# a-slide/Quade

Hardware: AMD Instinct MI355X
Metric: read-pairs/sec demultiplexed (2x150 bp, dual 8 bp index) (higher is better)
Workload: dtype u8

## Files before the change

### quade_amd/csrc/quade_deflate.hip

```cpp
#include <hip/hip_runtime.h>
#include <stdint.h>
#include <stdio.h>

#include "crc_lds.h"
#include "quade_deflate.h"

namespace {
constexpr int BLOCK = 256, TILE = BLOCK * 16;
constexpr uint32_t HEADER_BITS = 80 + 3 + 14 + 19 * 3 + 259 * 4;

__device__ uint32_t rev_bits(uint32_t v, int n) { return __brev(v) >> (32 - n); }

__device__ void code_lengths(const uint32_t* freq, int n, uint8_t* len, uint16_t* order , uint32_t* w , int16_t* parent ) {
    int m = 0;
    for (int s = 0; s < n; ++s) {
        len[s] = 0;
        if (freq[s]) order[m++] = (uint16_t)s;
    }
    for (int s = 0; m < 2 && s < n; ++s) {
        bool used = false;
        for (int i = 0; i < m; ++i) used |= order[i] == s;
        if (!used) order[m++] = (uint16_t)s;
    }
    auto f = [&](int s) -> uint32_t { return freq[s] ? freq[s] : 1u; };
    for (int i = 1; i < m; ++i) {
        const uint16_t s = order[i];
        int j = i - 1;
        while (j >= 0 && (f(order[j]) > f(s) || (f(order[j]) == f(s) && order[j] > s))) {
            order[j + 1] = order[j];
            --j;
        }
        order[j + 1] = s;
    }
    for (int i = 0; i < m; ++i) w[i] = f(order[i]);
    for (int i = 0; i < 2 * m - 1; ++i) parent[i] = -1;
    int leaf = 0, inner = m, next = m;
    while (next < 2 * m - 1) {
        int pick[2];
        for (int k = 0; k < 2; ++k) pick[k] = (leaf < m && (inner >= next || w[leaf] <= w[inner])) ? leaf++ : inner++;
        w[next] = w[pick[0]] + w[pick[1]];
        parent[pick[0]] = parent[pick[1]] = (int16_t)next;
        ++next;
    }
    int bl[16] = {0};
    w[2 * m - 2] = 0;
    for (int k = 2 * m - 3; k >= 0; --k) w[k] = w[parent[k]] + 1;
    for (int i = 0; i < m; ++i) ++bl[w[i] < 15 ? w[i] : 15];
    uint32_t kraft = 0;
    for (int d = 1; d <= 15; ++d) kraft += (uint32_t)bl[d] << (15 - d);
    for (uint32_t excess = kraft - (1u << 15); excess > 0; --excess) {
        int bits = 14;
        while (bl[bits] == 0) --bits;
        --bl[bits];
        bl[bits + 1] += 2;
        --bl[15];
    }
    int at = 0;
    for (int bits = 15; bits >= 1; --bits)
        for (int c = 0; c < bl[bits]; ++c) len[order[at++]] = (uint8_t)bits;
}

__global__ __launch_bounds__(BLOCK) void huff_pieces(const uint8_t* text, const qd_deflate_piece* pieces, uint8_t* out,
                                                     int64_t out_stride, uint32_t* out_bytes) {
    __shared__ uint32_t hist[4][4][256];
    __shared__ uint32_t freq[257];
    __shared__ uint32_t lut[257];
    __shared__ uint8_t len[257];
    __shared__ uint16_t order[257];
    __shared__ uint32_t wtmp[513];
    __shared__ int16_t parent[513];
    __shared__ uint32_t scan[BLOCK];
    __shared__ uint32_t words[TILE * 15 / 32 + 16];
    __shared__ uint32_t carry_word, carry_bits;
    const int tid = threadIdx.x, wave = tid >> 6, rep = tid & 3;
    const int64_t a = (int64_t)pieces[blockIdx.x].text_off, L = (int64_t)pieces[blockIdx.x].text_len;
    const uint8_t* src = text + a;
    uint32_t* dst = reinterpret_cast<uint32_t*>(out + (int64_t)blockIdx.x * out_stride);
    for (int i = tid; i < 4 * 4 * 256; i += BLOCK) (&hist[0][0][0])[i] = 0;
    __syncthreads();
    for (int64_t t = 0; t < L; t += TILE) {
        const int64_t p = t + (int64_t)tid * 16;
        if (p + 16 <= L) {
            const uint4 v = *reinterpret_cast<const uint4*>(src + p);
            const uint32_t q[4] = {v.x, v.y, v.z, v.w};
#pragma unroll
            for (int j = 0; j < 16; ++j) atomicAdd(&hist[wave][rep][(q[j >> 2] >> (8 * (j & 3))) & 0xff], 1u);
        } else {
            for (int64_t i = p; i < L; ++i) atomicAdd(&hist[wave][rep][src[i]], 1u);
        }
    }
    __syncthreads();
    for (int s = tid; s < 256; s += BLOCK) {
        uint32_t c = 0;
        for (int i = 0; i < 16; ++i) c += (&hist[0][0][0])[i * 256 + s];
        freq[s] = c;
    }
    if (tid == 0) freq[256] = 1;
    __syncthreads();
    if (tid == 0) {
        code_lengths(freq, 257, len, order, wtmp, parent);
        int blc[16] = {0}, nxt[16] = {0};
        for (int s = 0; s < 257; ++s) ++blc[len[s]];
        blc[0] = 0;
        for (int b = 1, c = 0; b <= 15; ++b) {
            c = (c + blc[b - 1]) << 1;
            nxt[b] = c;
        }
        for (int s = 0; s < 257; ++s) lut[s] = len[s] ? ((uint32_t)len[s] | (rev_bits((uint32_t)nxt[len[s]]++, len[s]) << 8)) : 0;
        uint64_t acc = 0;
        int cnt = 0, wi = 0;
        auto put = [&](uint32_t v, int n) {
            acc |= (uint64_t)v << cnt;
            cnt += n;
            if (cnt >= 32) {
                dst[wi++] = (uint32_t)acc;
                acc >>= 32;
                cnt -= 32;
            }
        };
        const uint8_t head[10] = {0x1f, 0x8b, 8, 0, 0, 0, 0, 0, 0, 0xff};
        for (int i = 0; i < 10; ++i) put(head[i], 8);
        put(1, 1);
        put(2, 2);
        put(0, 5);
        put(1, 5);
        put(15, 4);
        const uint8_t ord[19] = {16, 17, 18, 0, 8, 7, 9, 6, 10, 5, 11, 4, 12, 3, 13, 2, 14, 1, 15};
        for (int k = 0; k < 19; ++k) put(ord[k] < 16 ? 4 : 0, 3);
        for (int s = 0; s < 257; ++s) put(rev_bits(len[s], 4), 4);
        put(rev_bits(1, 4), 4);
        put(rev_bits(1, 4), 4);
        carry_word = (uint32_t)acc;
        carry_bits = (uint32_t)cnt;
        scan[0] = (uint32_t)wi;
        uint64_t bits = HEADER_BITS;
        for (int s = 0; s < 257; ++s) bits += (uint64_t)freq[s] * len[s];
        scan[1] = ((bits + 7) / 8 + 8 + 8 <= (uint64_t)out_stride) ? 1u : 0u;
    }
    __syncthreads();
    uint32_t out_word = scan[0];
    const bool fits = scan[1] != 0;
    __syncthreads();
    if (!fits) {
        if (tid == 0) out_bytes[blockIdx.x] = 0;
        return;
    }
    for (int64_t t = 0; t < L; t += TILE) {
        const int64_t p = t + (int64_t)tid * 16;
        uint32_t q[4] = {0, 0, 0, 0};
        int nbytes = 0;
        if (p + 16 <= L) {
            const uint4 v = *reinterpret_cast<const uint4*>(src + p);
            q[0] = v.x; q[1] = v.y; q[2] = v.z; q[3] = v.w;
            nbytes = 16;
        } else if (p < L) {
            nbytes = (int)(L - p);
            for (int i = 0; i < nbytes; ++i) q[i >> 2] |= (uint32_t)src[p + i] << (8 * (i & 3));
        }
        uint64_t b[4] = {0, 0, 0, 0};
        uint32_t nb = 0;
#pragma unroll
        for (int j = 0; j < 16; ++j) {
            if (j < nbytes) {
                const uint32_t e = lut[(q[j >> 2] >> (8 * (j & 3))) & 0xff];
                const uint64_t c = e >> 8;
                const uint32_t l = e & 0xff, wi = nb >> 6, sh = nb & 63;
                b[wi] |= c << sh;
                if (sh + l > 64 && wi < 3) b[wi + 1] |= c >> (64 - sh);
                nb += l;
            }
        }
        uint32_t x = nb;
#pragma unroll
        for (int d = 1; d < 64; d <<= 1) {
            const uint32_t y = __shfl_up(x, d, 64);
            if ((tid & 63) >= d) x += y;
        }
        if ((tid & 63) == 63) scan[wave] = x;
        __syncthreads();
        uint32_t base = 0, total = 0;
#pragma unroll
        for (int i = 0; i < BLOCK / 64; ++i) {
            const uint32_t v = scan[i];
            if (i < wave) base += v;
            total += v;
        }
        const uint32_t mine = base + x - nb;
        const uint32_t cb = carry_bits, cw = carry_word;
        const uint32_t nwords = (cb + total + 31) >> 5;
        for (uint32_t i = tid; i <= nwords; i += BLOCK) words[i] = i == 0 ? cw : 0;
        __syncthreads();
        if (nb) {
            const uint32_t pos = cb + mine, w0 = pos >> 5, sh = pos & 31;
            uint32_t prev = 0;
#pragma unroll
            for (int i = 0; i < 8; ++i) {
                const uint32_t d = (uint32_t)(b[i >> 1] >> (32 * (i & 1)));
                const uint32_t o = sh ? (d << sh) | (prev >> (32 - sh)) : d;
                if (o && 32u * i < nb + sh) atomicOr(&words[w0 + i], o);
                prev = d;
            }
            const uint32_t o = sh ? prev >> (32 - sh) : 0;
            if (o) atomicOr(&words[w0 + 8], o);
        }
        __syncthreads();
        const uint32_t full = (cb + total) >> 5;
        for (uint32_t i = tid; i < full; i += BLOCK) dst[out_word + i] = words[i];
        __syncthreads();
        if (tid == 0) {
            carry_word = words[full];
            carry_bits = (cb + total) & 31;
        }
        out_word += full;
        __syncthreads();
    }
    if (tid == 0) {
        uint64_t acc = carry_word;
        int cnt = (int)carry_bits;
        const uint32_t e = lut[256];
        acc |= (uint64_t)(e >> 8) << cnt;
        cnt += (int)(e & 0xff);
        uint8_t* bytes = reinterpret_cast<uint8_t*>(dst) + (size_t)out_word * 4;
        int nby = 0;
        while (cnt > 0) {
            bytes[nby++] = (uint8_t)acc;
            acc >>= 8;
            cnt -= 8;
        }
        const uint32_t c = pieces[blockIdx.x].crc32, isz = (uint32_t)L;
        for (int i = 0; i < 4; ++i) bytes[nby++] = (uint8_t)(c >> (8 * i));
        for (int i = 0; i < 4; ++i) bytes[nby++] = (uint8_t)(isz >> (8 * i));
        out_bytes[blockIdx.x] = out_word * 4 + (uint32_t)nby;
    }
}

}

hipError_t qd_launch_huffman(const uint8_t* text, const qd_deflate_piece* pieces, uint32_t n_pieces, uint8_t* out, int64_t out_stride,
                             uint32_t* out_bytes, hipStream_t st) {
    if (n_pieces == 0) return hipSuccess;
    hipLaunchKernelGGL(huff_pieces, dim3(n_pieces), dim3(BLOCK), 0, st, text, pieces, out, out_stride, out_bytes);
    return hipGetLastError();
}

namespace {
#ifndef QD_LZ_WAVES
#define QD_LZ_WAVES 8
#endif
constexpr int LZ_SUB = QD_LZ_SUB, LZ_WAVES = QD_LZ_WAVES, LZ_BLOCK = 64 * LZ_WAVES, LZ_REG = LZ_SUB / LZ_WAVES;
constexpr int LZ_HASH_BITS = 11, LZ_NICE = 32, LZ_DNA_MIN = 12, LZ_MATCH_BITS = 13, LZ_MAXLEN = 256;
constexpr int LZ_CRC_SW = LZ_WAVES >= 16 ? 17 : (LZ_WAVES >= 8 ? 33 : 65);
constexpr int LZ_TEXT_WORDS = (LZ_SUB + 320) / 4;
constexpr int LZ_NL = 286, LZ_ND = 30;
static_assert(LZ_SUB <= 65536 && LZ_SUB % 256 == 0, "table entries are 16-bit positions inside the sub-block");

__device__ __forceinline__ uint32_t rd32(const uint32_t* tw, uint32_t p) {
    const uint32_t i = p >> 2;
    return __builtin_amdgcn_alignbyte(tw[i + 1], tw[i], p & 3u);
}
__device__ __forceinline__ void rd256(const uint32_t* tw, uint32_t p, uint32_t (&a)[8]) {
    const uint32_t i = p >> 2, sh = p & 3u;
    uint32_t w[9];
#pragma unroll
    for (int k = 0; k < 9; ++k) w[k] = tw[i + k];
#pragma unroll
    for (int k = 0; k < 8; ++k) a[k] = __builtin_amdgcn_alignbyte(w[k + 1], w[k], sh);
}
__device__ __forceinline__ uint32_t same32(const uint32_t* tw, const uint32_t (&a)[8], uint32_t c) {
    uint32_t b[8];
    rd256(tw, c, b);
    uint32_t n = 32;
#pragma unroll
    for (int k = 7; k >= 0; --k) {
        const uint32_t x = a[k] ^ b[k];
        if (x) n = 4u * (uint32_t)k + ((uint32_t)__builtin_ctz(x) >> 3);
    }
    return n;
}
__device__ __forceinline__ bool bases4(uint32_t v) {
    return __builtin_amdgcn_perm(0x4E000000u, 0x47544341u, (v >> 1) & 0x07070707u) == v;
}
__device__ __forceinline__ void len_symbol(uint32_t l, uint32_t& sym, uint32_t& eb, uint32_t& ev) {
    if (l < 8) {
        sym = 257 + l;
        eb = ev = 0;
    } else if (l == 255) {
        sym = 285;
        eb = ev = 0;
    } else {
        const uint32_t n = 31u - (uint32_t)__clz(l);
        eb = n - 2;
        sym = 257 + 4 * (n - 1) + ((l >> eb) & 3u);
        ev = l & ((1u << eb) - 1);
    }
}
__device__ __forceinline__ void dist_symbol(uint32_t d, uint32_t& sym, uint32_t& eb, uint32_t& ev) {
    if (d < 4) {
        sym = d;
        eb = ev = 0;
    } else {
        const uint32_t n = 31u - (uint32_t)__clz(d);
        eb = n - 1;
        sym = 2 * n + ((d >> eb) & 1u);
        ev = d & ((1u << eb) - 1);
    }
}
__device__ __forceinline__ uint32_t len_extra_bits(uint32_t sym) {
    return (sym < 265 || sym == 285) ? 0u : (sym - 261) >> 2;
}
__device__ __forceinline__ uint32_t dist_extra_bits(uint32_t sym) { return sym < 4 ? 0u : (sym >> 1) - 1; }

__device__ void block_code_lengths(const uint32_t* freq, int n, uint8_t* len, uint32_t* fx, uint16_t* order, uint32_t* w, int16_t* parent,
                                   uint32_t* m_out) {
    __shared__ uint32_t bl[16];
    const int tid = threadIdx.x, nthr = blockDim.x;
    for (int s = tid; s < n; s += nthr) {
        fx[s] = freq[s];
        len[s] = 0;
    }
    if (tid < 16) bl[tid] = 0;
    if (tid == 0) *m_out = 0;
    __syncthreads();
    for (int s = tid; s < n; s += nthr)
        if (fx[s]) atomicAdd(m_out, 1u);
    __syncthreads();
    if (tid == 0 && *m_out < 2) {
        int used = (int)*m_out;
        for (int s = 0; used < 2 && s < n; ++s)
            if (!fx[s]) {
                fx[s] = 1;
                ++used;
            }
        *m_out = (uint32_t)used;
    }
    __syncthreads();
    const int m = (int)*m_out;
    for (int s = tid; s < n; s += nthr) {
        const uint32_t f = fx[s];
        if (!f) continue;
        int rank = 0;
        for (int t = 0; t < n; ++t) {
            const uint32_t g = fx[t];
            rank += (g != 0 && (g < f || (g == f && t < s))) ? 1 : 0;
        }
        order[rank] = (uint16_t)s;
        w[rank] = f;
    }
    for (int i = tid; i < 2 * m - 1; i += nthr) parent[i] = -1;
    __syncthreads();
    if (tid == 0) {
        int leaf = 0, inner = m, next = m;
        while (next < 2 * m - 1) {
            int pick[2];
            for (int k = 0; k < 2; ++k) pick[k] = (leaf < m && (inner >= next || w[leaf] <= w[inner])) ? leaf++ : inner++;
            w[next] = w[pick[0]] + w[pick[1]];
            parent[pick[0]] = parent[pick[1]] = (int16_t)next;
            ++next;
        }
    }
    __syncthreads();
    for (int i = tid; i < m; i += nthr) {
        uint32_t d = 0;
        for (int k = i; parent[k] >= 0; k = parent[k]) ++d;
        atomicAdd(&bl[d < 15 ? d : 15], 1u);
    }
    __syncthreads();
    if (tid == 0) {
        uint32_t kraft = 0;
        for (int d = 1; d <= 15; ++d) kraft += bl[d] << (15 - d);
        for (uint32_t excess = kraft - (1u << 15); excess > 0; --excess) {
            int bits = 14;
            while (bl[bits] == 0) --bits;
            --bl[bits];
            bl[bits + 1] += 2;
            --bl[15];
        }
    }
    __syncthreads();
    for (int i = tid; i < m; i += nthr) {
        int bits = 15;
        for (uint32_t upto = bl[15]; (uint32_t)i >= upto && bits > 1;) upto += bl[--bits];
        len[order[i]] = (uint8_t)bits;
    }
    __syncthreads();
}

__device__ void block_canonical_lut(const uint8_t* len, int n, uint32_t* lut) {
    __shared__ uint32_t cnt[16], nxt[16];
    const int tid = threadIdx.x, nthr = blockDim.x;
    if (tid < 16) cnt[tid] = 0;
    __syncthreads();
    for (int s = tid; s < n; s += nthr)
        if (len[s]) atomicAdd(&cnt[len[s]], 1u);
    __syncthreads();
    if (tid == 0) {
        uint32_t c = 0;
        for (int b = 1; b <= 15; ++b) {
            c = (c + (b > 1 ? cnt[b - 1] : 0u)) << 1;
            nxt[b] = c;
        }
    }
    __syncthreads();
    for (int s = tid; s < n; s += nthr) {
        const uint32_t l = len[s];
        uint32_t rank = 0;
        for (int t = 0; t < s; ++t) rank += len[t] == l ? 1u : 0u;
        lut[s] = l ? (l | (rev_bits(nxt[l] + rank, (int)l) << 8)) : 0u;
    }
    __syncthreads();
}

__device__ __forceinline__ void lds_barrier() { asm volatile("s_waitcnt lgkmcnt(0)\n\ts_barrier" ::: "memory"); }

#if defined(QD_LZ_TIMING)
__device__ unsigned long long g_lz_ticks[8];
#define LZ_STAMP(k)                                                          \
    do {                                                                     \
        __syncthreads();                                                     \
        const uint64_t now_ = (uint64_t)wall_clock64();                      \
        if (threadIdx.x == 0) atomicAdd(&g_lz_ticks[k], (unsigned long long)(now_ - since_)); \
        since_ = now_;                                                       \
    } while (0)
#else
#define LZ_STAMP(k) \
    do {            \
    } while (0)
#endif

__global__ __launch_bounds__(LZ_BLOCK) void lz_subblocks(const uint8_t* text, const qd_lz_sub* subs, uint32_t* tokens, uint8_t* sub_out,
                                                         int64_t sub_stride, uint32_t* sub_bytes, uint32_t* sub_crc) {
    extern __shared__ __attribute__((aligned(16))) uint8_t lz_lds[];
    uint32_t* tw = reinterpret_cast<uint32_t*>(lz_lds);
    uint32_t* table = reinterpret_cast<uint32_t*>(lz_lds + (size_t)LZ_TEXT_WORDS * 4);
    __shared__ uint32_t lfreq[288], dfreq[32], llut[288], dlut[32];
    __shared__ uint8_t llen[288], dlen[32], bcost[256];
    __shared__ uint32_t wave_ntok[LZ_WAVES], scan[LZ_WAVES], ctl[4];
    __shared__ uint32_t carry_word, carry_bits;
    const uint32_t tid = threadIdx.x, lane = tid & 63u, wave = tid >> 6;
    const uint32_t L = subs[blockIdx.x].text_len;
    const uint8_t* src = text + subs[blockIdx.x].text_off;
    uint32_t* dst = reinterpret_cast<uint32_t*>(sub_out + (int64_t)blockIdx.x * sub_stride);
    uint32_t* tok0 = tokens + (size_t)blockIdx.x * LZ_SUB;
#if defined(QD_LZ_TIMING)
    uint64_t since_ = (uint64_t)wall_clock64();
#endif

    static_assert((1u << LZ_HASH_BITS) == 8 * 256, "the byte histogram's replicas borrow the hash table's space");
    for (uint32_t i = tid; i < (1u << LZ_HASH_BITS); i += LZ_BLOCK) table[i] = 0;
    for (uint32_t i = tid; i < 288; i += LZ_BLOCK) lfreq[i] = 0;
    if (tid < 32) dfreq[tid] = 0;
    __syncthreads();
    for (uint32_t i = tid; i < (uint32_t)LZ_TEXT_WORDS / 4; i += LZ_BLOCK) {
        uint4 v = make_uint4(0, 0, 0, 0);
        const uint32_t b = i * 16;
        if (b + 16 <= L) {
            v = *reinterpret_cast<const uint4*>(src + b);
        } else if (b < L) {
            uint32_t q[4] = {0, 0, 0, 0};
            for (uint32_t k = b; k < L; ++k) q[(k - b) >> 2] |= (uint32_t)src[k] << (8 * ((k - b) & 3));
            v = make_uint4(q[0], q[1], q[2], q[3]);
        }
        reinterpret_cast<uint4*>(tw)[i] = v;
        if (b < L) {
            const uint32_t q[4] = {v.x, v.y, v.z, v.w}, nby = min(16u, L - b);
            uint32_t* rep = table + (tid & 7u);
#pragma unroll
            for (uint32_t k = 0; k < 16; ++k)
                if (k < nby) atomicAdd(&rep[((q[k >> 2] >> (8 * (k & 3))) & 0xFFu) << 3], 1u);
        }
    }
    __syncthreads();
    if (tid < 256) {
        uint32_t h = 0;
#pragma unroll
        for (int r = 0; r < 8; ++r) h += table[(tid << 3) + r];
        const int c = h ? (int)(__log2f((float)L / (float)h) + 0.5f) : 12;
        bcost[tid] = (uint8_t)(c < 1 ? 1 : (c > 12 ? 12 : c));
    }
    __syncthreads();
    LZ_STAMP(0);
    if (sub_crc) {
        static_assert((4u << LZ_HASH_BITS) >= 4096 + 64 && (size_t)LZ_BLOCK * LZ_CRC_SW * 4 >= (size_t)LZ_SUB, "the CRC stage's tables and slices");
        qdcrc::stage_tables<LZ_BLOCK>(table);
        __syncthreads();
        const uint32_t crc = qdcrc::crc32_lds<LZ_BLOCK, LZ_CRC_SW>(tw, L, table, table + 1024);
        if (tid == 0) sub_crc[blockIdx.x] = crc;
    }
    for (uint32_t i = tid; i < (1u << LZ_HASH_BITS); i += LZ_BLOCK) table[i] = 0;
    __syncthreads();
    LZ_STAMP(1);

    for (uint32_t r0 = 0; r0 < L; r0 += LZ_BLOCK) {
        const uint32_t p = r0 + tid;
        uint32_t ins_h = 0xFFFFFFFFu, ins_v = 0;
        if (p < L) {
            uint32_t a[8];
            rd256(tw, p, a);
            uint32_t best = 0, dist = 0;
            if (p + 4 <= L) {
                const uint32_t h = (a[0] * 2654435761u) >> (32 - LZ_HASH_BITS);
                const uint32_t bucket = table[h];
                if (p >= 1 && rd32(tw, p - 1) == a[0]) {
                    best = same32(tw, a, p - 1);
                    dist = 1;
                }
#pragma unroll
                for (int k = 0; k < 2; ++k) {
                    const uint32_t c = (bucket >> (16 * k)) & 0xFFFFu;
                    uint32_t n = 0;
                    if (c < p && rd32(tw, c) == a[0]) n = same32(tw, a, c);
                    if (c < p && p - c <= 32768u && n > best) {
                        best = n;
                        dist = p - c;
                    }
                }
                best = min(best, L - p);
                const uint32_t need = (bases4(a[0]) && bases4(a[1])) ? (uint32_t)LZ_DNA_MIN : 4u;
                if (best < need) {
                    best = 0;
                } else {
                    uint32_t c8 = 0;
#pragma unroll
                    for (int k = 0; k < 8; ++k) c8 += bcost[(a[k >> 2] >> (8 * (k & 3))) & 0xFFu];
                    const uint32_t mbits = (uint32_t)LZ_MATCH_BITS + (dist > 1 ? 31u - (uint32_t)__clz(dist) : 0u);
                    if (best * c8 < mbits * 8) best = 0;
                }
#if defined(QD_LZ_RACY)
                table[h] = (bucket << 16) | p;
#else
                ins_h = h;
                ins_v = (bucket << 16) | p;
#endif
            }
            tok0[p] = best | (dist << 8);
        }
        lds_barrier();
#if !defined(QD_LZ_RACY)
        if (ins_h != 0xFFFFFFFFu) atomicMax(&table[ins_h], ins_v);
        lds_barrier();
#endif
    }
    __syncthreads();

    LZ_STAMP(2);
    {
        const uint32_t rbeg = wave * LZ_REG, rend = min(rbeg + (uint32_t)LZ_REG, L);
        uint32_t* tok = tok0 + rbeg;
        uint32_t ntok = 0;
        int carry = 0;
        constexpr uint32_t AHEAD = (1u << LZ_HASH_BITS) / LZ_WAVES / 64;
        static_assert(AHEAD >= 1 && AHEAD * 64 * LZ_WAVES == (1u << LZ_HASH_BITS), "the waves' shares of the table's space");
        uint32_t* cbuf = table + wave * (AHEAD * 64);
        uint32_t in_buf = AHEAD;
        for (uint32_t base = rbeg; base < rend; base += 64) {
            const uint32_t p = base + lane;
            const int limit = (int)min(64u, rend - base);
            uint32_t eff = 0, dist = 0;
            if (in_buf == AHEAD) {
#pragma unroll
                for (uint32_t j = 0; j < AHEAD; ++j) cbuf[64 * j + lane] = p + 64 * j < rend ? tok0[p + 64 * j] : 0u;
                in_buf = 0;
            }
            const uint32_t cd = cbuf[64 * in_buf + lane];
            ++in_buf;
            if ((int)lane < limit) {
                eff = min(cd & 0xFFu, rend - p);
                dist = cd >> 8;
                if (eff < 4) eff = 0;
            }
            const uint32_t lit = (tw[p >> 2] >> (8 * (p & 3u))) & 0xFFu;
            const uint32_t eff_next = (uint32_t)__shfl_down((int)eff, 1, 64);
            const bool deferred = eff != 0 && (int)lane + 1 < limit && eff_next > eff && eff < (uint32_t)LZ_NICE;
            const uint64_t mm = __ballot(eff != 0 && !deferred);
            const uint64_t xm = __ballot(eff >= (uint32_t)LZ_NICE && !deferred);
            uint32_t tlen = eff;
            const uint32_t tdist = dist;
            uint64_t starts = 0;
            int s = carry;
            while (s < limit) {
                if ((mm >> s) & 1ull) {
                    uint32_t len = (uint32_t)__builtin_amdgcn_readlane((int)eff, s);
                    if ((xm >> s) & 1ull) {
                        const uint32_t D = (uint32_t)__builtin_amdgcn_readlane((int)dist, s);
                        const uint32_t ps = base + (uint32_t)s;
                        const uint32_t x = rd32(tw, ps + 4 * lane) ^ rd32(tw, ps - D + 4 * lane);
                        const uint64_t nz = __ballot(x != 0);
                        len = LZ_MAXLEN;
                        if (nz) {
                            const int fl = __builtin_ctzll(nz);
                            const uint32_t xf = (uint32_t)__builtin_amdgcn_readlane((int)x, fl);
                            len = 4u * (uint32_t)fl + ((uint32_t)__builtin_ctz(xf) >> 3);
                        }
                        len = min(len, rend - ps);
                        if ((int)lane == s) tlen = len;
                    }
                    starts |= 1ull << s;
                    s += (int)len;
                } else {
                    const uint64_t rest = (mm >> s) << s;
                    int nxt = rest ? __builtin_ctzll(rest) : 64;
                    if (nxt > limit) nxt = limit;
                    const uint64_t upto = nxt >= 64 ? ~0ull : ((1ull << nxt) - 1);
                    starts |= upto & ~((1ull << s) - 1);
                    s = nxt;
                }
            }
            if (!((mm >> lane) & 1ull)) tlen = 0;
            carry = s - 64;
            if ((starts >> lane) & 1ull) {
                uint32_t t;
                if (tlen) {
                    t = (tlen - 3) | ((tdist - 1) << 8);
                    uint32_t sym, eb, ev;
                    len_symbol(tlen - 3, sym, eb, ev);
                    atomicAdd(&lfreq[sym], 1u);
                    dist_symbol(tdist - 1, sym, eb, ev);
                    atomicAdd(&dfreq[sym], 1u);
                } else {
                    t = 0x80000000u | lit;
                    atomicAdd(&lfreq[lit], 1u);
                }
                tok[ntok + (uint32_t)__popcll(starts & ((1ull << lane) - 1))] = t;
            }
            ntok += (uint32_t)__popcll(starts);
        }
        if (lane == 0) wave_ntok[wave] = ntok;
    }
    if (tid == 0) lfreq[256] = 1;
    __syncthreads();
    LZ_STAMP(3);

    {
        uint32_t* fx = tw;
        uint16_t* order = reinterpret_cast<uint16_t*>(tw + 288);
        uint32_t* w = tw + 288 + 144;
        int16_t* parent = reinterpret_cast<int16_t*>(tw + 288 + 144 + 576);
        block_code_lengths(lfreq, LZ_NL, llen, fx, order, w, parent, &ctl[2]);
        block_code_lengths(dfreq, LZ_ND, dlen, fx, order, w, parent, &ctl[2]);
    }
    LZ_STAMP(4);
    uint32_t* words = tw + 2048;
    block_canonical_lut(llen, LZ_NL, llut);
    block_canonical_lut(dlen, LZ_ND, dlut);
    if (tid == 0) ctl[3] = 0;
    __syncthreads();
    {
        uint32_t bits = 0;
        for (uint32_t s = tid; s < (uint32_t)LZ_NL; s += LZ_BLOCK) bits += lfreq[s] * (llen[s] + (s > 256 ? len_extra_bits(s) : 0u));
        for (uint32_t s = tid; s < (uint32_t)LZ_ND; s += LZ_BLOCK) bits += dfreq[s] * (dlen[s] + dist_extra_bits(s));
        if (bits) atomicAdd(&ctl[3], bits);
    }
    __syncthreads();
    LZ_STAMP(7);
    if (tid == 0) {
        int nl = LZ_NL, nd = LZ_ND;
        while (nl > 257 && llen[nl - 1] == 0) --nl;
        while (nd > 1 && dlen[nd - 1] == 0) --nd;
        uint64_t acc = 0;
        int cnt = 0, wi = 0;
        auto put = [&](uint32_t v, int n) {
            acc |= (uint64_t)v << cnt;
            cnt += n;
            if (cnt >= 32) {
                dst[wi++] = (uint32_t)acc;
                acc >>= 32;
                cnt -= 32;
            }
        };
        put(0, 1);
        put(2, 2);
        put((uint32_t)(nl - 257), 5);
        put((uint32_t)(nd - 1), 5);
        put(15, 4);
        const uint8_t ord[19] = {16, 17, 18, 0, 8, 7, 9, 6, 10, 5, 11, 4, 12, 3, 13, 2, 14, 1, 15};
        for (int k = 0; k < 19; ++k) put(ord[k] == 0 ? 2u : ((ord[k] == 17 || ord[k] == 18) ? 3u : 5u), 3);
        auto len_at = [&](int i) -> uint32_t { return i < nl ? llen[i] : dlen[i - nl]; };
        auto put_len = [&](uint32_t v) { put(rev_bits(15u + v, 5), 5); };
        const int nseq = nl + nd;
        for (int i = 0; i < nseq;) {
            const uint32_t v = len_at(i);
            int run = 1;
            while (i + run < nseq && len_at(i + run) == v) ++run;
            i += run;
            if (v == 0) {
                while (run >= 11) {
                    const int r = run < 138 ? run : 138;
                    put(6, 3);
                    put((uint32_t)(r - 11), 7);
                    run -= r;
                }
                if (run >= 3) {
                    put(2, 3);
                    put((uint32_t)(run - 3), 3);
                    run = 0;
                }
                for (; run > 0; --run) put(0, 2);
            } else {
                put_len(v);
                --run;
                while (run >= 3) {
                    const int r = run < 6 ? run : 6;
                    put_len(16);
                    put((uint32_t)(r - 3), 2);
                    run -= r;
                }
                for (; run > 0; --run) put_len(v);
            }
        }
        carry_word = (uint32_t)acc;
        carry_bits = (uint32_t)cnt;
        const uint64_t bits = 3 + 14 + 19 * 3 + 5 * (uint64_t)(nl + nd) + ctl[3];
        ctl[0] = (uint32_t)wi;
        ctl[1] = ((bits + 7) / 8 + 3 + 4 + 8 <= (uint64_t)sub_stride) ? 1u : 0u;
    }
    __syncthreads();
    LZ_STAMP(5);
    uint32_t out_word = ctl[0];
    if (ctl[1] == 0) {
        if (tid == 0) sub_bytes[blockIdx.x] = 0;
        return;
    }
    constexpr int LZ_TPL = 4;
    uint32_t pre[LZ_WAVES + 1];
    pre[0] = 0;
#pragma unroll
    for (int i = 0; i < LZ_WAVES; ++i) pre[i + 1] = pre[i] + wave_ntok[i];
    const uint32_t T = pre[LZ_WAVES];
    for (uint32_t g0 = 0; g0 < T; g0 += LZ_BLOCK * LZ_TPL) {
        uint32_t t[LZ_TPL];
#pragma unroll
        for (int j = 0; j < LZ_TPL; ++j) {
            const uint32_t g = g0 + tid * LZ_TPL + j;
            t[j] = 0;
            if (g < T) {
                uint32_t wv = 0;
#pragma unroll
                for (int i = 1; i < LZ_WAVES; ++i) wv += g >= pre[i] ? 1u : 0u;
                t[j] = tok0[(size_t)wv * LZ_REG + (g - pre[wv])];
            }
        }
        uint64_t b[LZ_TPL];
        uint32_t nb[LZ_TPL], mine = 0;
#pragma unroll
        for (int j = 0; j < LZ_TPL; ++j) {
            b[j] = 0;
            nb[j] = 0;
            if (g0 + tid * LZ_TPL + j < T) {
                if (t[j] & 0x80000000u) {
                    const uint32_t e = llut[t[j] & 0xFFu];
                    b[j] = e >> 8;
                    nb[j] = e & 0xFFu;
                } else {
                    uint32_t sym, eb, ev;
                    len_symbol(t[j] & 0xFFu, sym, eb, ev);
                    uint32_t e = llut[sym];
                    b[j] = (uint64_t)(e >> 8) | ((uint64_t)ev << (e & 0xFFu));
                    nb[j] = (e & 0xFFu) + eb;
                    dist_symbol((t[j] >> 8) & 0x7FFFu, sym, eb, ev);
                    e = dlut[sym];
                    b[j] |= ((uint64_t)(e >> 8) | ((uint64_t)ev << (e & 0xFFu))) << nb[j];
                    nb[j] += (e & 0xFFu) + eb;
                }
            }
            mine += nb[j];
        }
        uint32_t x = mine;
#pragma unroll
        for (int d = 1; d < 64; d <<= 1) {
            const uint32_t y = __shfl_up(x, d, 64);
            if (lane >= (uint32_t)d) x += y;
        }
        if (lane == 63) scan[wave] = x;
        lds_barrier();
        uint32_t before = 0, total = 0;
#pragma unroll
        for (int i = 0; i < LZ_WAVES; ++i) {
            const uint32_t v = scan[i];
            if ((uint32_t)i < wave) before += v;
            total += v;
        }
        const uint32_t cb = carry_bits, cw = carry_word;
        const uint32_t nwords = (cb + total + 31) >> 5;
        for (uint32_t i = tid; i <= nwords + 2; i += LZ_BLOCK) words[i] = i == 0 ? cw : 0;
        lds_barrier();
        uint32_t pos = cb + before + x - mine;
#pragma unroll
        for (int j = 0; j < LZ_TPL; ++j) {
            if (nb[j]) {
                const uint32_t w0 = pos >> 5, sh = pos & 31u;
                const uint64_t lo = b[j] << sh;
                const uint32_t hi = sh ? (uint32_t)(b[j] >> (64 - sh)) : 0u;
                if ((uint32_t)lo) atomicOr(&words[w0], (uint32_t)lo);
                if ((uint32_t)(lo >> 32)) atomicOr(&words[w0 + 1], (uint32_t)(lo >> 32));
                if (hi) atomicOr(&words[w0 + 2], hi);
            }
            pos += nb[j];
        }
        lds_barrier();
        const uint32_t full = (cb + total) >> 5;
        for (uint32_t i = tid; i < full; i += LZ_BLOCK) dst[out_word + i] = words[i];
        if (tid == 0) {
            carry_word = words[full];
            carry_bits = (cb + total) & 31u;
        }
        out_word += full;
    }
    __syncthreads();
    LZ_STAMP(6);
    if (tid == 0) {
        uint64_t acc = carry_word;
        int cnt = (int)carry_bits;
        const uint32_t e = llut[256];
        acc |= (uint64_t)(e >> 8) << cnt;
        cnt += (int)(e & 0xFFu);
        cnt += 3;
        uint8_t* bytes = reinterpret_cast<uint8_t*>(dst) + (size_t)out_word * 4;
        int nby = 0;
        while (cnt > 0) {
            bytes[nby++] = (uint8_t)acc;
            acc >>= 8;
            cnt -= 8;
        }
        bytes[nby++] = 0;
        bytes[nby++] = 0;
        bytes[nby++] = 0xFF;
        bytes[nby++] = 0xFF;
        sub_bytes[blockIdx.x] = out_word * 4 + (uint32_t)nby;
    }
}

__global__ __launch_bounds__(256) void lz_members(const qd_deflate_piece* pieces, const qd_lz_sub* subs, const uint32_t* first_sub, uint32_t n_subs,
                                                  const uint8_t* sub_out, int64_t sub_stride, const uint32_t* sub_bytes, uint8_t* out,
                                                  int64_t out_stride, uint32_t* out_bytes) {
    const bool empty = blockIdx.x >= n_subs;
    const uint32_t piece = empty ? blockIdx.x - n_subs : subs[blockIdx.x].piece;
    const uint32_t j0 = first_sub[piece], j1 = first_sub[piece + 1], j = blockIdx.x;
    if (empty && j1 != j0) return;
    uint64_t total = 10 + 2 + 8, off = 10;
    bool ok = true;
    for (uint32_t k = j0; k < j1; ++k) {
        const uint32_t n = sub_bytes[k];
        ok = ok && n > 0;
        total += n;
        if (k < j) off += n;
    }
    const bool first = empty || j == j0, last = empty || j + 1 == j1;
    if (!ok || total > (uint64_t)out_stride) {
        if (first && threadIdx.x == 0) out_bytes[piece] = 0;
        return;
    }
    uint8_t* dst = out + (int64_t)piece * out_stride;
    if (!empty) {
        const uint32_t n = sub_bytes[j];
        const uint8_t* s = sub_out + (int64_t)j * sub_stride;
        for (uint32_t k = threadIdx.x; k < n; k += 256) dst[off + k] = s[k];
        off += n;
    }
    if (threadIdx.x == 0) {
        if (first) {
            const uint8_t head[10] = {0x1f, 0x8b, 8, 0, 0, 0, 0, 0, 0, 0xff};
            for (int i = 0; i < 10; ++i) dst[i] = head[i];
        }
        if (last) {
            dst[off++] = 0x03;
            dst[off++] = 0x00;
            const uint32_t c = pieces[piece].crc32, isz = pieces[piece].text_len;
            for (int i = 0; i < 4; ++i) dst[off++] = (uint8_t)(c >> (8 * i));
            for (int i = 0; i < 4; ++i) dst[off++] = (uint8_t)(isz >> (8 * i));
            out_bytes[piece] = (uint32_t)off;
        }
    }
}
}

hipError_t qd_launch_lz_subblocks(const uint8_t* text, const qd_lz_sub* subs, uint32_t n_subs, uint32_t* tokens, uint8_t* sub_out, int64_t sub_stride,
                                  uint32_t* sub_bytes, uint32_t* sub_crc, hipStream_t st) {
    if (n_subs == 0) return hipSuccess;
    constexpr size_t lds = (size_t)LZ_TEXT_WORDS * 4 + (4u << LZ_HASH_BITS);
    static_assert(LZ_TEXT_WORDS % 4 == 0, "the text is staged 16 bytes at a time");
    hipError_t e = hipFuncSetAttribute(reinterpret_cast<const void*>(lz_subblocks), hipFuncAttributeMaxDynamicSharedMemorySize, (int)lds);
    if (e != hipSuccess) return e;
    hipLaunchKernelGGL(lz_subblocks, dim3(n_subs), dim3(LZ_BLOCK), lds, st, text, subs, tokens, sub_out, sub_stride, sub_bytes, sub_crc);
#if defined(QD_LZ_TIMING)
    {
        unsigned long long t[8];
        (void)hipStreamSynchronize(st);
        (void)hipMemcpyFromSymbol(t, HIP_SYMBOL(g_lz_ticks), sizeof t);
        static const char* names[8] = {"stage+histogram", "crc", "candidates", "parse", "code lengths", "header (one lane)", "encode", "tables"};
        unsigned long long sum = 0;
        for (int k = 0; k < 8; ++k) sum += t[k];
        fprintf(stderr, "lz_subblocks phases (all launches so far, %u sub-blocks in this one):", n_subs);
        for (int k = 0; k < 8; ++k) fprintf(stderr, " %s %.1f %%", names[k], sum ? 100.0 * (double)t[k] / (double)sum : 0.0);
        fprintf(stderr, "\n");
    }
#endif
    return hipGetLastError();
}

hipError_t qd_launch_lz_members(const qd_deflate_piece* pieces, uint32_t n_pieces, const qd_lz_sub* subs, const uint32_t* first_sub, uint32_t n_subs,
                                const uint8_t* sub_out, int64_t sub_stride, const uint32_t* sub_bytes, uint8_t* out, int64_t out_stride, uint32_t* out_bytes,
                                hipStream_t st) {
    if (n_pieces == 0) return hipSuccess;
    hipLaunchKernelGGL(lz_members, dim3(n_subs + n_pieces), dim3(256), 0, st, pieces, subs, first_sub, n_subs, sub_out, sub_stride, sub_bytes,
                       out, out_stride, out_bytes);
    return hipGetLastError();
}

hipError_t qd_launch_lz(const uint8_t* text, const qd_deflate_piece* pieces, uint32_t n_pieces, const qd_lz_sub* subs, const uint32_t* first_sub,
                        uint32_t n_subs, uint32_t* tokens, uint8_t* sub_out, int64_t sub_stride, uint32_t* sub_bytes, uint8_t* out,
                        int64_t out_stride, uint32_t* out_bytes, hipStream_t st) {
    if (n_pieces == 0) return hipSuccess;
    const hipError_t e = qd_launch_lz_subblocks(text, subs, n_subs, tokens, sub_out, sub_stride, sub_bytes, nullptr, st);
    if (e != hipSuccess) return e;
    return qd_launch_lz_members(pieces, n_pieces, subs, first_sub, n_subs, sub_out, sub_stride, sub_bytes, out, out_stride, out_bytes, st);
}
```

Before: 181.0 billion.

## Emit the dynamic Huffman header with one wavefront instead of one lane

The per-sub-block deflate header (code-length run-length encoding) was built serially by thread 0. It is now built by wave 0: ballots find the trimmed table sizes and run starts, each run-start lane computes its piece bit count, and a packed 12-bit wave prefix scan assigns bit positions. Lanes then atomicOr their bits into a zeroed LDS word buffer, which is copied out to the destination. This removes a long single-lane serial phase in exchange for more LDS atomics and register use, and relies on the packed prefix fields not overflowing.

Result: no change. 179.8 billion (-0.7%).

```diff
diff --git a/quade_amd/csrc/quade_deflate.hip b/quade_amd/csrc/quade_deflate.hip
--- a/quade_amd/csrc/quade_deflate.hip
+++ b/quade_amd/csrc/quade_deflate.hip
@@ -408,6 +408,40 @@
         lut[s] = l ? (l | (rev_bits(nxt[l] + rank, (int)l) << 8)) : 0u;
     }
     __syncthreads();
+}
+
+constexpr int LZ_HDR_PER_LANE = (LZ_NL + LZ_ND + 1 + 63) / 64, LZ_HDR_WORDS = 64;
+static_assert(LZ_HDR_PER_LANE * 12 <= 64 && 5 * (LZ_NL + LZ_ND) < (1 << 12), "a lane's bit counts are the 12-bit fields of one 64-bit scan");
+static_assert((17 + 57 + 5 * (LZ_NL + LZ_ND) + 31) / 32 + 1 <= LZ_HDR_WORDS && LZ_HDR_WORDS <= LZ_BLOCK, "the header's words (at most 5 bits per length)");
+__device__ constexpr uint64_t hdr_code_length_code() {
+    constexpr uint8_t ord[19] = {16, 17, 18, 0, 8, 7, 9, 6, 10, 5, 11, 4, 12, 3, 13, 2, 14, 1, 15};
+    uint64_t bits = 0;
+    for (int k = 0; k < 19; ++k) bits |= (uint64_t)(ord[k] == 0 ? 2u : ((ord[k] == 17 || ord[k] == 18) ? 3u : 5u)) << (3 * k);
+    return bits;
+}
+template <class F>
+__device__ __forceinline__ void hdr_run_pieces(uint32_t v, uint32_t run, F&& f) {
+    if (v == 0) {
+        while (run >= 11) {
+            const uint32_t r = min(run, 138u);
+            f(6u | ((r - 11u) << 3), 10u);
+            run -= r;
+        }
+        if (run >= 3)
+            f(2u | ((run - 3u) << 3), 6u);
+        else if (run)
+            f(0u, 2u * run);
+    } else {
+        const uint32_t own = rev_bits(15u + v, 5);
+        f(own, 5u);
+        --run;
+        while (run >= 3) {
+            const uint32_t r = min(run, 6u);
+            f(31u | ((r - 3u) << 5), 7u);
+            run -= r;
+        }
+        if (run) f(run == 2 ? own | (own << 5) : own, 5u * run);
+    }
 }
 
 __device__ __forceinline__ void lds_barrier() { asm volatile("s_waitcnt lgkmcnt(0)\n\ts_barrier" ::: "memory"); }
@@ -643,6 +677,7 @@
     block_canonical_lut(llen, LZ_NL, llut);
     block_canonical_lut(dlen, LZ_ND, dlut);
     if (tid == 0) ctl[3] = 0;
+    if (tid < LZ_HDR_WORDS) words[tid] = 0;
     __syncthreads();
     {
         uint32_t bits = 0;
@@ -652,66 +687,82 @@
     }
     __syncthreads();
     LZ_STAMP(7);
-    if (tid == 0) {
-        int nl = LZ_NL, nd = LZ_ND;
-        while (nl > 257 && llen[nl - 1] == 0) --nl;
-        while (nd > 1 && dlen[nd - 1] == 0) --nd;
-        uint64_t acc = 0;
-        int cnt = 0, wi = 0;
-        auto put = [&](uint32_t v, int n) {
-            acc |= (uint64_t)v << cnt;
-            cnt += n;
-            if (cnt >= 32) {
-                dst[wi++] = (uint32_t)acc;
-                acc >>= 32;
-                cnt -= 32;
-            }
-        };
-        put(0, 1);
-        put(2, 2);
-        put((uint32_t)(nl - 257), 5);
-        put((uint32_t)(nd - 1), 5);
-        put(15, 4);
-        const uint8_t ord[19] = {16, 17, 18, 0, 8, 7, 9, 6, 10, 5, 11, 4, 12, 3, 13, 2, 14, 1, 15};
-        for (int k = 0; k < 19; ++k) put(ord[k] == 0 ? 2u : ((ord[k] == 17 || ord[k] == 18) ? 3u : 5u), 3);
-        auto len_at = [&](int i) -> uint32_t { return i < nl ? llen[i] : dlen[i - nl]; };
-        auto put_len = [&](uint32_t v) { put(rev_bits(15u + v, 5), 5); };
-        const int nseq = nl + nd;
-        for (int i = 0; i < nseq;) {
-            const uint32_t v = len_at(i);
-            int run = 1;
-            while (i + run < nseq && len_at(i + run) == v) ++run;
-            i += run;
-            if (v == 0) {
-                while (run >= 11) {
-                    const int r = run < 138 ? run : 138;
-                    put(6, 3);
-                    put((uint32_t)(r - 11), 7);
-                    run -= r;
+    if (wave == 0) {
+        const uint64_t lm = __ballot(lane < 29u && llen[257u + lane] != 0);
+        const uint64_t dm = __ballot(lane >= 1u && lane < 30u && dlen[lane] != 0);
+        const uint32_t nl = 257u + (lm ? 64u - (uint32_t)__builtin_clzll(lm) : 0u);
+        const uint32_t nd = dm ? 64u - (uint32_t)__builtin_clzll(dm) : 1u;
+        const uint32_t nseq = nl + nd;
+        auto len_at = [&](uint32_t i) -> uint32_t { return i < nl ? llen[i] : (i < nseq ? dlen[i - nl] : 0xFFu); };
+        uint32_t v[LZ_HDR_PER_LANE], run[LZ_HDR_PER_LANE];
+        uint64_t starts[LZ_HDR_PER_LANE];
+#pragma unroll
+        for (int j = 0; j < LZ_HDR_PER_LANE; ++j) {
+            const uint32_t i = 64u * j + lane;
+            v[j] = len_at(i);
+            starts[j] = __ballot(v[j] != (i ? len_at(i - 1) : 0xFEu));
+        }
+        uint64_t counts = 0;
+#pragma unroll
+        for (int j = 0; j < LZ_HDR_PER_LANE; ++j) {
+            const uint32_t i = 64u * j + lane;
+            run[j] = 0;
+            if (i < nseq && ((starts[j] >> lane) & 1ull)) {
+                uint32_t next = 0;
+                bool found = false;
+#pragma unroll
+                for (int w = j; w < LZ_HDR_PER_LANE; ++w) {
+                    const uint64_t m = w == j ? starts[w] & ~((2ull << lane) - 1ull) : starts[w];
+                    if (!found && m) {
+                        next = 64u * w + (uint32_t)__builtin_ctzll(m);
+                        found = true;
+                    }
                 }
-                if (run >= 3) {
-                    put(2, 3);
-                    put((uint32_t)(run - 3), 3);
-                    run = 0;
-                }
-                for (; run > 0; --run) put(0, 2);
-            } else {
-                put_len(v);
-                --run;
-                while (run >= 3) {
-                    const int r = run < 6 ? run : 6;
-                    put_len(16);
-                    put((uint32_t)(r - 3), 2);
-                    run -= r;
-                }
-                for (; run > 0; --run) put_len(v);
-            }
-        }
-        carry_word = (uint32_t)acc;
-        carry_bits = (uint32_t)cnt;
-        const uint64_t bits = 3 + 14 + 19 * 3 + 5 * (uint64_t)(nl + nd) + ctl[3];
-        ctl[0] = (uint32_t)wi;
-        ctl[1] = ((bits + 7) / 8 + 3 + 4 + 8 <= (uint64_t)sub_stride) ? 1u : 0u;
+                run[j] = next - i;
+                uint32_t nb = 0;
+                hdr_run_pieces(v[j], run[j], [&](uint32_t, uint32_t n) { nb += n; });
+                counts |= (uint64_t)nb << (12 * j);
+            }
+        }
+        uint64_t x = counts;
+#pragma unroll
+        for (int d = 1; d < 64; d <<= 1) {
+            const uint64_t y = __shfl_up(x, d, 64);
+            if (lane >= (uint32_t)d) x += y;
+        }
+        const uint64_t totals = __shfl(x, 63, 64);
+        uint32_t base = 17 + 57;
+#pragma unroll
+        for (int j = 0; j < LZ_HDR_PER_LANE; ++j) {
+            if (run[j]) {
+                uint32_t pos = base + (uint32_t)((x >> (12 * j)) & 0xFFFu) - (uint32_t)((counts >> (12 * j)) & 0xFFFu);
+                hdr_run_pieces(v[j], run[j], [&](uint32_t bits, uint32_t n) {
+                    if (bits) {
+                        const uint64_t lo = (uint64_t)bits << (pos & 31u);
+                        atomicOr(&words[pos >> 5], (uint32_t)lo);
+                        if ((uint32_t)(lo >> 32)) atomicOr(&words[(pos >> 5) + 1], (uint32_t)(lo >> 32));
+                    }
+                    pos += n;
+                });
+            }
+            base += (uint32_t)((totals >> (12 * j)) & 0xFFFu);
+        }
+        if (lane == 0) {
+            const uint64_t lo = 0u | (2u << 1) | ((nl - 257u) << 3) | ((nd - 1u) << 8) | (15u << 13) | (hdr_code_length_code() << 17);
+            atomicOr(&words[0], (uint32_t)lo);
+            atomicOr(&words[1], (uint32_t)(lo >> 32));
+            atomicOr(&words[2], (uint32_t)(hdr_code_length_code() >> 47));
+        }
+        asm volatile("s_waitcnt lgkmcnt(0)" ::: "memory");
+        const uint32_t wi = base >> 5;
+        for (uint32_t i = lane; i < wi; i += 64) dst[i] = words[i];
+        if (lane == 0) {
+            carry_word = words[wi];
+            carry_bits = base & 31u;
+            const uint64_t bits = 3 + 14 + 19 * 3 + 5 * (uint64_t)(nl + nd) + ctl[3];
+            ctl[0] = wi;
+            ctl[1] = ((bits + 7) / 8 + 3 + 4 + 8 <= (uint64_t)sub_stride) ? 1u : 0u;
+        }
     }
     __syncthreads();
     LZ_STAMP(5);
@@ -886,12 +937,12 @@
         unsigned long long t[8];
         (void)hipStreamSynchronize(st);
         (void)hipMemcpyFromSymbol(t, HIP_SYMBOL(g_lz_ticks), sizeof t);
-        static const char* names[8] = {"stage+histogram", "crc", "candidates", "parse", "code lengths", "header (one lane)", "encode", "tables"};
+        static const char* names[8] = {"stage+histogram", "crc", "candidates", "parse", "code lengths", "header", "encode", "tables"};
         unsigned long long sum = 0;
         for (int k = 0; k < 8; ++k) sum += t[k];
         fprintf(stderr, "lz_subblocks phases (all launches so far, %u sub-blocks in this one):", n_subs);
         for (int k = 0; k < 8; ++k) fprintf(stderr, " %s %.1f %%", names[k], sum ? 100.0 * (double)t[k] / (double)sum : 0.0);
-        fprintf(stderr, "\n");
+        fprintf(stderr, "; sum %.2f s of workgroup time\n", (double)sum / 1e8);
     }
 #endif
     return hipGetLastError();
```
